# Li-Jinjie/ndp_nmpc_qd

Measured on AMD Instinct MI355X. Metric: NMPC solves/sec (N=20, 1 RTI iter + downwash MLP) at batch, higher is better.
Workload: dtype f64

## Files before the change

### ndp_nmpc_qd_amd/csrc/host.hpp

```cpp
#pragma once
#include <hip/hip_runtime.h>

#include <atomic>
#include <cstdint>
#include <memory>
#include <mutex>
#include <string>
#include <vector>

#include "wave_gfx950.hpp"
#include "cfg_params.hpp"
#include "kern_args.hpp"
#include "rti_table.hpp"
#include "hip_own.hpp"

#define NDP_HIDDEN __attribute__((visibility("hidden")))

using namespace ndp;

struct ndp_handle {
    Stream stream, aux;
    ndp_cfg cfg;
    RtiParams P;
    int lds_per_wave = 0;
    int waves = 4;
    int n_simd = 1024;
    mutable std::atomic<uint64_t> rti_launched{0};
    bool use_queue = false;
    bool queue_auto = false;
    PinnedBuf<unsigned long long> hIpm;
    unsigned long long ipm_seen = 0, steps_seen = 0;
    unsigned queue_launches = 0;
    double *dX = nullptr, *dU = nullptr;
    double *sx0 = nullptr, *sxr = nullptr, *sur = nullptr, *sother = nullptr, *sego = nullptr, *su0 = nullptr;
    float *sf = nullptr;
    int *dStatus = nullptr, *dIters = nullptr;
    const int *lastStatus = nullptr, *lastIters = nullptr;
    double *dRingU = nullptr;
    DevBuf<float> dForce, dFrag;
    DevBuf<double> dKC;
    DevBuf<int> dTables;
    DevBuf<signed char> dAct;
    int sens_level = 0;
    DevBuf<double> dSensU0, dSensU, dSensX;
    DevBuf<double> dPSensXr, dPSensUr, dPSensF;
    DevBuf<double> dVjp;
    DevBuf<int> dVjpSt;
    DevBuf<signed char> dVjpAct;
    DevBuf<double> dClWs;
    DevBuf<int> dFormIndex;
    int form_K = 0, form_edges = 0;
    DevBuf<double> dFormWs;
    DevBuf<float> dFragT, dGwPart;
    DevBuf<float> dFitPart;
    DevBuf<unsigned long long> dTrain;
    DevBuf<double> dThr;
    DevBuf<double> dStamps;
    DevBuf<double> dTraj;
    int traj_seg = 0;
    DevBuf<double> dRingX;
    unsigned long long list_n = 0;
    int segc_par = 0;
    int list_step = 5;
    DevBuf<int> dTickIndex;
    DevBuf<double> dTickThrust;
    bool tick_gate = true;
    const double *tick_remote = nullptr;
    int tick_remote_stride = 6;
    struct TickSlot { bool busy = false, want_u0 = false; } tslot[2];
    DevBuf<double> dRelay;
    DevBuf<double> sThr;
    DevBuf<float> dForceAB[2];
    DevBuf<unsigned long long> dProto;
    Event evFork, evJoin;
    unsigned prefetch_timeout_us = 100000, pf_groups_rti = 1, pf_ntiles = 1;
    DevBuf<unsigned> dQctr;
    DevBuf<int> dQids;
    bool have_mlp = false;
    DevBuf<unsigned char> dIn, dOut;
// ... 185 lines not shown
```

### ndp_nmpc_qd_amd/csrc/kern_args.hpp

```cpp
#pragma once
#include <hip/hip_runtime.h>

#include <stddef.h>

#include <type_traits>

#include "wave_gfx950.hpp"
#include "rti_wave.hpp"

namespace ndp {

struct ThrCfg { double a1, a2, hm, g, R, Q0, Q1, mass; };

struct RingGeom {
    int step, np1;
    __host__ __device__ int ring() const { return step * (np1 - 1) + 1; }
    __host__ __device__ size_t px() const { return (size_t)step * 2 * np1 * 10; }
    __host__ __device__ size_t pu() const { return (size_t)step * 2 * np1 * 4; }
    __host__ __device__ size_t slot(unsigned long long j) const { return (size_t)(j % step) * 2 * np1 + (size_t)((j / step) % np1); }
};

struct RefCfg { int B, N, n_seg; double dt, mass, g, toff; };

struct TickPre {
    RefCfg cf;
    const double *coeff, *tcum, *tseg, *fpt;
    int *seg_hint;
    const double *t;
    double t_all;
    int advance;
    unsigned long long j_new;
    RingGeom rg;
    double *rx, *ru;
    ThrCfg thr;
    double *st;
    const double *vz;
    size_t vz_pitch;
    const double *throttle;
    int est;
    double *pv = nullptr;
    size_t pv_slot = 0;
};

struct BatchPtrs {
    const double *kc;
    const int *tables;
    const double *x0, *xr, *ur;
    const float *f;
    double *X, *U, *u0;
    int *status, *iters;
    double *Xm, *Um;
    double *dbg;
    double *stamps;
    size_t xr_pitch, ur_pitch;
    size_t x0_pitch;
    double *cmd;
    const double *kthr;
    double *thrust_keep;
    double cmd_mass;
    int f_f64;
    signed char *act;
};

struct MlpArgs {
    const float *frag;
    const double *other;
    const double *ego_xy;
    float *force_out;
    double r2;
    int other_stride;
    const int *other_index;
    int other_sys;
    size_t other_pitch;
    size_t ego_pitch;
};

struct QueueArgs {
    unsigned *count;
    int *ids;
    unsigned long long *ipm_total;
};

enum { PF_GROUPS = 8, PF_STRIDE = 512, PF_CUR_M = 0, PF_RTI_C1 = 1 * PF_STRIDE, PF_RTI_C2 = 9 * PF_STRIDE,
       PF_MISSED = 10 * PF_STRIDE, PF_GATE_TIMEOUT = 11 * PF_STRIDE, PF_MLP_DONE = 12 * PF_STRIDE, PF_SLOW = 13 * PF_STRIDE, PF_EPOCH = 14 * PF_STRIDE  };
struct LateArgs {
    unsigned long long *proto;
    const float *F[2];
    unsigned timeout_us;
    unsigned groups_rti, ntiles;
};
__device__ __host__ inline unsigned pf_group_size(unsigned n, unsigned groups, unsigned g) { return n / groups + (g < n % groups ? 1u : 0u); }

enum { SEGC_SLOT = 32, SEGC_PER = 72 };
struct TickArgs {
    const double *coeff, *tcum, *tseg, *fpt;
    const double *segc;
    double *segc_wr;
    int n_seg;
    const double *t;
    double t_all;
    int advance;
    double toff, mass, g;
    unsigned long long j_new;
    size_t new_slot;
    RingGeom rg;
    double *rx, *ru;
    ThrCfg thr;
    double *st;
    const double *vz;
    size_t vz_pitch;
    const double *throttle;
    int est;
};

struct KernArgs {
    RtiParams P;
    BatchPtrs bp;
    int B, lds_per_wave;
    MlpArgs ma;
    QueueArgs qa;
    LateArgs la;
    TickArgs ta;
};
struct SensArgs {
    double *du0 = nullptr, *dU = nullptr, *dX = nullptr;
    int level = 0;
};
// ... 19 lines not shown
```

### ndp_nmpc_qd_amd/csrc/mlp_tile.hpp

```cpp
#pragma once
#include <hip/hip_runtime.h>

#include "mlp_common.hpp"

namespace ndp {

typedef __attribute__((address_space(3))) float *lds_f32;
typedef const __attribute__((address_space(3))) float *lds_cf32;

enum { FR_L1 = 0, FR_B1 = FR_L1 + 12 * 64, FR_B2 = FR_B1 + 128, FR_B3 = FR_B2 + 64, FR_W4 = FR_B3 + 128,
       FR_B4 = FR_W4 + 4 * 128, FR_HF = FR_B4 + 4, FR_REC = 2 * 64 * 8 / 2 ,
       FR_USED = FR_HF + 32 * FR_REC,
       FR_CHUNKS = (FR_USED + 2047) / 2048 * 8, FR_TOTAL = FR_CHUNKS * 256 };
static_assert(FR_HF % 4 == 0 && FR_W4 % 4 == 0, "16-byte alignment of the LDS image");
static_assert(FR_L1 == frag::L1 && FR_B1 == frag::B1 && FR_B2 == frag::B2 && FR_B3 == frag::B3 && FR_W4 == frag::W4 && FR_B4 == frag::B4 &&
              FR_HF == frag::HF && FR_REC == frag::REC && FR_TOTAL == frag::TOTAL, "mlp_common.hpp: frag:: restates this enum for mlp_vjp.hip");


__device__ __forceinline__ void stage_fragments(const float *__restrict__ fr, lds_f32 dst, int tid, int nthreads)
{
    const int wave = __builtin_amdgcn_readfirstlane(tid >> 6), lane = tid & 63, nw = nthreads >> 6;
#pragma unroll
    for (int i = 0; i < FR_CHUNKS; ++i) {
        if (i * nw >= FR_CHUNKS) break;
        const int c = wave + i * nw;
        if ((i + 1) * nw <= FR_CHUNKS || c < FR_CHUNKS)
            __builtin_amdgcn_global_load_lds((const __attribute__((address_space(1))) void *)(fr + c * 256 + lane * 4),
                                             (__attribute__((address_space(3))) void *)(dst + c * 256), 16, 0, 0);
    }
}

__device__ __forceinline__ void load_w(lds_cf32 fr, int rec, int lane, Split2 &w)
{
    const __attribute__((address_space(3))) h16x8 *p = (const __attribute__((address_space(3))) h16x8 *)(fr + FR_HF) + rec * 128 + lane;
    w.hi = p[0]; w.lo = p[64];
}

__device__ __forceinline__ void mlp_tile(lds_cf32 fr, const float zb[3], int lane, float o[3])
{
    typedef float f4_t __attribute__((ext_vector_type(4)));
    const int h = lane >> 5;
    Split2 x1[4][2], x2[2][2];
    f16_t h3[4];
    float bc[16];
#pragma unroll
    for (int ot = 0; ot < 4; ++ot) {
#pragma unroll
        for (int r = 0; r < 16; ++r) bc[r] = fr[FR_B1 + ot * 32 + f0(r) + 4 * h];
        f16_t acc;
#pragma unroll
        for (int r = 0; r < 16; ++r) acc[r] = bc[r];
#pragma unroll
        for (int s = 0; s < 3; ++s)
            acc = __builtin_amdgcn_mfma_f32_32x32x2f32(fr[FR_L1 + (ot * 3 + s) * 64 + lane], zb[s], acc, 0, 0, 0);
#pragma unroll
        for (int r = 0; r < 16; ++r) acc[r] = relu_cap(acc[r]);
        split2(acc, 0, x1[ot][0]);
        split2(acc, 1, x1[ot][1]);
    }
    Split2 wc, wn;
    load_w(fr, 0, lane, wc);
    f16_t acc, accl;
#pragma unroll
    for (int rec = 0; rec < 32; ++rec) {
        const bool l2 = rec < 16;
        const int q = l2 ? rec : rec - 16;
        const int ot = l2 ? q / 8 : q / 4, it = l2 ? (q / 2) % 4 : (q / 2) % 2, s = q % 2;
        const bool first = l2 ? (q % 8 == 0) : (q % 4 == 0), last = l2 ? (q % 8 == 7) : (q % 4 == 3);
        if (rec + 1 < 32) load_w(fr, rec + 1, lane, wn);
        if (first) {
#pragma unroll
            for (int r = 0; r < 16; ++r) {
                acc[r] = fr[(l2 ? FR_B2 : FR_B3) + ot * 32 + f0(r) + 4 * h];
                accl[r] = 0.0f;
            }
        }
#ifdef NDP_DEV_HALF_TILE
        if (!(rec & 1))
#endif
        mm3(wc, l2 ? x1[it][s] : x2[it][s], acc, accl);
        if (last) {
#pragma unroll
            for (int r = 0; r < 16; ++r) {
                const float v = fmaf(accl[r], NDP_LO_INV, acc[r]);
                acc[r] = l2 ? relu_cap(v) : fmaxf(v, 0.0f);
            }
            if (l2) { split2(acc, 0, x2[ot][0]); split2(acc, 1, x2[ot][1]); }
            else h3[ot] = acc;
        }
        wc = wn;
    }
    const __attribute__((address_space(3))) f4_t *w4 = (const __attribute__((address_space(3))) f4_t *)(fr + FR_W4);
    f4_t qc[16], qn[16];
#pragma unroll
    for (int r = 0; r < 16; ++r) qc[r] = w4[f0(r) + 4 * h];
    o[0] = o[1] = o[2] = 0.0f;
#pragma unroll
    for (int it = 0; it < 4; ++it) {
        if (it + 1 < 4) {
#pragma unroll
            for (int r = 0; r < 16; ++r) qn[r] = w4[(it + 1) * 32 + f0(r) + 4 * h];
        }
#pragma unroll
        for (int r = 0; r < 16; ++r) {
#pragma unroll
            for (int c = 0; c < 3; ++c) o[c] = fmaf(qc[r][c], h3[it][r], o[c]);
        }
#pragma unroll
        for (int r = 0; r < 16; ++r) qc[r] = qn[r];
    }
#pragma unroll
    for (int c = 0; c < 3; ++c) o[c] = o[c] + __shfl_xor(o[c], 32, 64) + fr[FR_B4 + c];
}

}
```

### ndp_nmpc_qd_amd/csrc/ndp_hip.hip

```cpp
#include <hip/hip_runtime.h>
#include <hip/hip_ext.h>

#include <sched.h>
#include <stdio.h>

#include <atomic>
#include <chrono>
#include <condition_variable>
#include <cstdlib>
#include <cstring>
#include <memory>
#include <mutex>
#include <new>
#include <string>
#include <thread>
#include <type_traits>
#include <vector>

#include "host.hpp"
#include "cond_qp.hpp"
#include "mlp_tile.hpp"

namespace ndp {

__global__ void queue_reset_kernel(unsigned *count, unsigned long long *ipm_total)
{
    if (threadIdx.x == 0) {
        *ipm_total += *count;
        *count = 0u;
    }
}

}

using namespace ndp;

struct PackJob { unsigned char *dst; const unsigned char *src; size_t len; size_t rows = 0, src_stride = 0; };
enum : size_t { PACK_CHUNK = (size_t)256 << 10 };
struct PackPool {
    std::vector<std::thread> th;
    std::mutex mu;
    std::condition_variable cv;
    std::atomic<const PackJob *> jobs{nullptr};
    std::atomic<int> njobs{0}, next{0}, active{0};
    std::unique_ptr<std::atomic<int>[]> done;
    int done_cap = 0;
    uint64_t gen = 0;
    std::atomic<uint64_t> gen_pub{0};
    bool stop = false;
    static void cpu_relax()
    {
#if !defined(__HIP_DEVICE_COMPILE__) && (defined(__x86_64__) || defined(__i386__))
        __asm__ __volatile__("pause");
#endif
    }

    explicit PackPool(int n)
    {
        for (int i = 0; i < n; ++i) th.emplace_back([this] { work(); });
    }
    ~PackPool()
    {
        { std::lock_guard<std::mutex> lk(mu); stop = true; }
        cv.notify_all();
        for (auto &t : th) t.join();
    }
    bool take_one()
    {
        const int n = njobs.load(std::memory_order_acquire);
        if (n == 0) return false;
        const int i = next.fetch_add(1, std::memory_order_acq_rel);
        if (i >= n) return false;
        const PackJob &j = jobs.load(std::memory_order_relaxed)[i];
        if (j.rows == 0) memcpy(j.dst, j.src, j.len);
// ... 120 lines not shown

int ndp_create(const ndp_cfg *cfg, ndp_handle **out)
{
    if (!cfg || !out) { g_create_err = "ndp_create: null argument"; return -1; }
    *out = nullptr;
    if (cfg->batch < 1 || cfg->N < 2 || slots_for(cfg->N) > 5 || cfg->n_rti < 1 || cfg->qp_precision < 0 || cfg->qp_precision > 6 ||
        cfg->work_queue < 0 || cfg->work_queue > 2 || !(cfg->ts_nmpc > 0.0) || cfg->dt < cfg->ts_nmpc) {
        g_create_err = "ndp_create: need batch >= 1, 2 <= N <= 46, n_rti >= 1, qp_precision in 0..6, work_queue in 0..2, 0 < ts_nmpc <= dt";
        return -2;
    }
    if (cfg->qp_precision >= 5 && (cfg->N % 4 != 0 || cfg->N > 40)) {
        g_create_err = "ndp_create: the condensed study (qp_precision 5 / 6) tiles the 4N x 4N Hessian by 16: N must be a multiple of 4, at most 40";
        return -2;
    }
    if (!as_gamma_holds(*cfg, cfg->Rd)) {
        g_create_err = "ndp_create: as_gamma must be finite and at least 1e8 * max(dt * Rd) when as_iter_max > 0 (a weaker pin does not hold "
                       "its input on the bound)";
        return -2;
    }
    if (cfg->ipm_refine > 0 && (slots_for(cfg->N) > 3 || cfg->qp_precision != 0)) {
        g_create_err = "ndp_create: ipm_refine > 0 is not served for this shape: the refinement path (stiff sweeps + second solves while a STATE bound's "
                       "barrier term exceeds refine_gamma) lives in the three-slot fp64 kernels only (N <= 27, qp_precision 0); the five-slot kernels "
                       "(N >= 28) sit at the register limit without it.  Set ipm_refine = 0: strongly active state bounds at a tight tolerance then "
                       "end in status 4 (never a silent answer)";
        return -2;
    }
    {
        const double ratio = cfg->dt / cfg->ts_nmpc, nearest = (double)(long long)(ratio + 0.5);
        if (ratio - nearest > 1e-9 || nearest - ratio > 1e-9) {
            g_create_err = "ndp_create: dt must be a whole multiple of ts_nmpc (node spacing = every k-th entry of the reference list)";
            return -2;
        }
    }
    int ndev = 0;
    hipError_t e = hipGetDeviceCount(&ndev);
    if (e != hipSuccess || ndev <= cfg->device) {
        g_create_err = std::string("ndp_create: no usable HIP device (") + hipGetErrorString(e) + ")";
        return -3;
    }
    ndp_handle *h = new (std::nothrow) ndp_handle;
    if (!h) return -4;
    h->cfg = *cfg;
    h->P = to_params(*cfg);
    h->list_step = (int)(cfg->dt / cfg->ts_nmpc + 0.5);
    h->lds_per_wave = (lds_doubles(cfg->N) + 1) & ~1;
    if (cfg->qp_precision >= 5) h->lds_per_wave += (cond_extra_doubles(cfg->N) + 1) & ~1;
    const size_t per_wave_bytes = (size_t)h->lds_per_wave * sizeof(double);
    h->waves = 4;
    while (h->waves > 1 && per_wave_bytes * h->waves > 160 * 1024) h->waves >>= 1;
    if (const char *e = getenv("NDP_DEV_WAVES")) {
        const int w = atoi(e);
        if ((w == 1 || w == 2 || w == 4) && w <= h->waves) h->waves = w;
    }
    auto fail = [&](const char *what, hipError_t err) {
        g_create_err = std::string("ndp_create: ") + what + ": " + hipGetErrorString(err);
        ndp_destroy(h);
        return -5;
    };
    if ((e = hipSetDevice(cfg->device)) != hipSuccess) return fail("hipSetDevice", e);
    {
        hipDeviceProp_t prop;
        if ((e = hipGetDeviceProperties(&prop, cfg->device)) != hipSuccess) return fail("hipGetDeviceProperties", e);
        h->n_simd = 4 * prop.multiProcessorCount;
    }
    if (cfg->work_queue == 1 && !(queue_shape(h) && cfg->qp_mode == NDP_QP_AUTO)) {
        g_create_err = "ndp_create: work_queue = 1 needs qp_mode AUTO, qp_precision 0 and (N, n_rti) = (20, 1) or (40, 2)";
        delete h;
        return -2;
    }
    h->queue_auto = cfg->work_queue == 0 && queue_shape(h) && cfg->qp_mode == NDP_QP_AUTO && cfg->N == 20 && cfg->batch >= 2 * h->n_simd;
    h->use_queue = cfg->work_queue == 1 || (cfg->work_queue == 0 && queue_shape(h) && cfg->qp_mode == NDP_QP_AUTO && cfg->N == 40);
    if (h->queue_auto) {
        if ((e = h->hIpm.alloc(64)) != hipSuccess) return fail("hipHostMalloc (work-list counter)", e);
        h->hIpm[0] = h->hIpm[1] = 0;
    }
    if ((e = h->stream.ensure(hipStreamNonBlocking)) != hipSuccess) return fail("hipStreamCreate", e);
    if ((e = h->evLast.ensure(hipEventDisableTiming)) != hipSuccess) return fail("hipEventCreate", e);
    const size_t B = cfg->batch;
    {
        size_t o = 0;
        h->off_x0 = o; o += up256(B * NX * 8);
        h->off_xr = o; o += up256(nxs(h) * 8);
        h->off_ur = o; o += up256(nus(h) * 8);
        h->off_f = o; o += up256(nfs(h) * 8);
        h->off_other = o; o += up256(nxs(h) * 8);
        h->off_ego = o; o += up256(B * 2 * 8);
        h->in_bytes = o;
        o = 0;
        h->off_u0 = o; o += up256(B * NU * 8);
        h->off_st = o; o += up256(B * 4);
        h->off_it = o; o += up256(B * 4);
        h->out_bytes = o;
        h->out_all = h->out_bytes + (nxs(h) + nus(h)) * 8;
    }
    std::string what;
    auto dev = [&](auto &buf, size_t bytes, const char *name) {
        if ((e = buf.alloc(bytes)) != hipSuccess) what = std::string("hipMalloc ") + name;
        return e == hipSuccess;
    };
    if (!dev(h->dForce, nfs(h) * 4, "dForce") || !dev(h->dFrag, FR_TOTAL * 4, "dFrag") || !dev(h->dFragT, FRT_TOTAL * 4, "dFragT") ||
        !dev(h->dGwPart, (size_t)mlp_vjp_groups(h) * NDP_MLP_NPARAM * 4, "dGwPart") || !dev(h->dKC, KC_HOST * 8, "dKC") ||
        !dev(h->dThr, B * 8 * 8, "dThr") || !dev(h->sThr, B * 11 * 8, "sThr") || !dev(h->dRelay, B * 4 * 8, "dRelay") ||
        !dev(h->dQctr, 256, "dQctr") || !dev(h->dQids, B * 4, "dQids") || !dev(h->dAct, act_bytes(h), "dAct") ||
        !dev(h->dTrain, TRAIN_WS_BYTES, "dTrain") ||
        !dev(h->dFitPart, FIT_WS_BYTES, "dFitPart") ||
        !dev(h->dTables, TB_WORDS * 4, "dTables") || !dev(h->dIn, h->in_bytes, "dIn") || !dev(h->dOut, h->out_all, "dOut") ||
// ... 104 lines not shown
    const int N = h->cfg.N, W = h->waves, pr = h->cfg.qp_precision, wi = W == 4 ? 0 : W == 2 ? 1 : 2;
    const bool ref = N == 20 && h->cfg.n_rti == 1;
    if (pr) {
        if (pr >= 3 && N == 40 && h->cfg.n_rti == 2 && W == 2) return pr == 3 ? K40_F32 : K40_BF16;
        return (RtiId)(KPREC1 + pr - 1);
    }
    if (h->sens_level > 0) {
        RtiId id;
        if (phase) id = phase == 2 ? S20_CONS : fused ? S20F_PROD : S20_PROD;
        else if (N == 20 && W == 4) id = fused ? S20F : S20;
        else if (W == 4) id = fused ? SF_4 : S_4;
        else id = fused ? SF_2 : S_2;
        if (!h->dPSensXr) return id;
        switch (id) {
        case S20F_PROD: return P20F_PROD;
        case S20_PROD: return P20_PROD;
        case S20_CONS: return P20_CONS;
        case S20F: return P20F;
        case S20: return P20;
        case SF_4: return PF_4;
        default: return PF_2;
        }
    }
    if (phase == 2) return N == 20 ? K20_CONS : K40_CONS;
    if (phase == 1) {
        if (N != 20) return K40_PROD;
        if (tick) return fused ? K20F_PROD_TICK : K20_PROD_TICK;
        return fused ? K20F_PROD : K20_PROD;
    }
    if (ref && W == 4) {
        if (tick) return fused ? K20F_TICK : K20_TICK;
        return fused ? K20F : prefetched ? K20_LATE : K20;
    }
    if (ref && W == 2) return fused ? K20F_W2 : K20_W2;
    if (N == 40 && h->cfg.n_rti == 2 && W == 2 && !fused) return K40;
    if (fused) return (RtiId)(K3F_4 + wi);
    return (RtiId)((slots_for(N) <= 3 ? K3_4 : K5_4) + wi);
}

int launch_rti(ndp_handle *h, const double *d_x0, const double *d_xr, const double *d_ur, const float *d_f,
               double *d_u0, double *d_dbg, hipStream_t s, const Neigh *nb, const StepOut *so, bool prefetched)
{
    int *d_status = so && so->status ? so->status : h->dStatus, *d_iters = so && so->iters ? so->iters : h->dIters;
    h->lastStatus = d_status; h->lastIters = d_iters;
    BatchPtrs bp{h->dKC, h->dTables, d_x0, d_xr, d_ur, d_f, h->dX, h->dU, d_u0, d_status, d_iters,
                 so ? so->Xm : nullptr, so ? so->Um : nullptr, d_dbg, h->dStamps,
                 so && so->xr_pitch ? so->xr_pitch : (size_t)(h->cfg.N + 1) * NX, so && so->ur_pitch ? so->ur_pitch : (size_t)h->cfg.N * NU, (size_t)NX,
                 so ? so->cmd : nullptr, so ? so->kthr : nullptr, so ? so->thrust_keep : nullptr, h->cfg.mass, so && so->f_f64 ? 1 : 0,
                 h->dAct};
    const bool fused = nb && nb->other;
    MlpArgs ma{fused ? h->dFrag : nullptr, fused ? nb->other : nullptr, fused ? nb->ego_xy : nullptr, h->dForce,
               h->cfg.r_horiz * h->cfg.r_horiz, fused ? nb->stride : NX, fused ? nb->index : nullptr, fused ? peer_mapped(nb->other) : 0,
               fused && nb->pitch ? nb->pitch : (size_t)(h->cfg.N + 1) * (fused ? nb->stride : NX), fused && nb->ego_pitch ? nb->ego_pitch : (size_t)2};
    QueueArgs qa{h->dQctr, h->dQids, reinterpret_cast<unsigned long long *>(h->dQctr + 16)};
    LateArgs la{prefetched ? h->dProto : nullptr, {h->dForceAB[0], h->dForceAB[1]}, h->prefetch_timeout_us,
                h->pf_groups_rti, h->pf_ntiles};
    KernArgs ka{h->P, bp, h->cfg.batch, h->lds_per_wave, ma, qa, la, so && so->tick ? *so->tick : TickArgs{}};
    SensArgs sa{h->dSensU0, h->sens_level >= 2 ? h->dSensU : nullptr, h->sens_level >= 2 ? h->dSensX : nullptr, h->sens_level};
    const bool tick1 = so && so->tick;
    const int pr = h->cfg.qp_precision;
    const bool q = h->use_queue && !d_dbg && !prefetched;
    h->last_step_tracked = false;
    if (h->track_steps) {
        hipStreamCaptureStatus cs = hipStreamCaptureStatusNone;
        if (hipStreamIsCapturing(s, &cs) != hipSuccess) { (void)hipGetLastError(); cs = hipStreamCaptureStatusNone; }
        if (cs != hipStreamCaptureStatusNone) {
            h->err = "tracked control steps (ndp_track_steps) cannot be launched on a stream that is being captured: switch tracking off "
                     "and order the exchange through the stream (ndp_xchg_begin's after_stream)";
            return -15;
        }
    }
    int rc = begin_timing(h, s, 0, true);
    if (rc) return rc;
    const bool ext_timing = h->timing_open && !q && !pr && !(so && so->done) && !h->track_steps;
    if (h->timing_open && !ext_timing) NDP_HIP(h, hipEventRecord(h->events.back().a, s));
    if (pr && fused) { h->err = "qp_precision != 0 supports f / no disturbance only (run ndp_downwash first)"; return -12; }
    hipEvent_t stop = nullptr;
    if (so && so->done) stop = so->done;
    else if (h->track_steps) { stop = h->stepDone[++h->step_seq & 3]; h->last_step_tracked = true; }
    if (h->sens_level > 0 && (prefetched || tick1)) { h->err = "launch_rti: the late-force and tick forms have no sensitivity kernel"; return -2; }
    launch_kern(h, rti_pick(h, fused, tick1, prefetched, q ? 1 : 0), s, ka, sa, ext_timing ? h->events.back().a : nullptr,
                ext_timing ? h->events.back().b : q || pr ? nullptr : stop);
    if (ext_timing) h->timing_open = false;
    NDP_HIP(h, hipGetLastError());
    if (q) {
        KernArgs kc = ka;
        kc.bp.f = fused ? h->dForce : d_f;
        kc.ma.frag = nullptr; kc.ma.other = nullptr;
        if (h->cfg.n_rti == 1 && h->cfg.as_iter_max <= 0) kc.P.qp_mode = QP_IPM_ALWAYS;
        launch_kern(h, rti_pick(h, fused, tick1, prefetched, 2), s, kc, sa);
        NDP_HIP(h, hipGetLastError());
        if (stop) hipExtLaunchKernelGGL(queue_reset_kernel, dim3(1), dim3(64), 0, s, nullptr, stop, 0, h->dQctr.get(), qa.ipm_total);
        else hipLaunchKernelGGL(queue_reset_kernel, dim3(1), dim3(64), 0, s, h->dQctr, qa.ipm_total);
        NDP_HIP(h, hipGetLastError());
    } else if (pr && stop) NDP_HIP(h, hipEventRecord(stop, s));
    const int rce = end_timing(h, s);
    queue_policy(h, s);
    return rce;
}

bool can_fuse(const ndp_handle *h)
{
    return h->cfg.qp_precision == 0 && h->cfg.N + 1 <= 32 && slots_for(h->cfg.N) <= 3 &&
           (size_t)h->lds_per_wave * sizeof(double) * h->waves >= FR_TOTAL * sizeof(float);
}

// ... 669 lines not shown
```

### ndp_nmpc_qd_amd/csrc/rti_kernel_body.inc

```
    static_assert(!(FUSED && QMODE == 2), "the consumer reads the force the producer left in global memory");
    static_assert(!TICK || (QMODE <= 1 && NC > 0 && PREC == 0), "the one-launch tick exists for the compile-time horizon's in-place and producer forms");
#ifndef NDP_NO_KERNARG_WARM
    {
        typedef const __attribute__((address_space(4))) unsigned *kptr;
        kptr kp = (kptr)__builtin_amdgcn_kernarg_segment_ptr();
        unsigned acc = 0;
#pragma unroll
        for (unsigned o = 0; o < (unsigned)sizeof(KernArgs); o += 64) acc |= kp[o / 4];
        asm volatile("" : : "s"(acc));
    }
#endif
    const RtiParams &P = ka.P;
    const BatchPtrs &bp = ka.bp;
    const MlpArgs &ma = ka.ma;
    const QueueArgs &qa = ka.qa;
    const int B = ka.B;
    const int wave = (int)(threadIdx.x >> 6);
    if (!FUSED && (QMODE == 0 || QMODE == 3) && ka.la.proto) {
        if (threadIdx.x == 0) wg_done = 0;
        __syncthreads();
    }
    int inst_raw = __builtin_amdgcn_readfirstlane((int)blockIdx.x * WAVES + wave);
    if (QMODE == 2) {
        const int n = (int)*qa.count;
        if (inst_raw >= n) return;
        inst_raw = __builtin_amdgcn_readfirstlane(qa.ids[inst_raw]);
    }
    const bool active = inst_raw < B;
    if (!FUSED && !active) return;
    const int inst = active ? inst_raw : B - 1;
    const int N = NC ? NC : P.N;
    const size_t nf = (size_t)(N + 1) * 3;
    RtiIo io;
    bind_instance(io, bp, inst, N);
    if (NSLOT <= 3 && (QMODE == 0 || QMODE == 3)) io.ipm_ctr = qa.ipm_total;
    if (NSLOT <= 3 && QMODE != 2 && blockIdx.x == 0 && threadIdx.x == 0 && qa.ipm_total)
        __hip_atomic_fetch_add(qa.ipm_total + 1, 1ull, __ATOMIC_RELAXED, __HIP_MEMORY_SCOPE_AGENT);
    if (!FUSED && (QMODE == 0 || QMODE == 3) && ka.la.proto) {
        const LateArgs &la = ka.la;
        const unsigned long long t = la.proto[PF_RTI_C2] / la.groups_rti + 1;
        const unsigned g = blockIdx.x % la.groups_rti;
        const unsigned np1 = (unsigned)N + 1, row0 = (unsigned)inst * np1;
        io.f_late = la.F[t & 1] + (size_t)inst * nf;
        io.late_flag = la.proto + PF_EPOCH + (t & 1) * la.ntiles + row0 / 32;
        io.late_flag2 = la.proto + PF_EPOCH + (t & 1) * la.ntiles + (row0 + np1 - 1) / 32;
        io.late_want = t;
        io.late_ready = la.proto[PF_MLP_DONE] >= t ? 1 : 0;
        io.late_timeout_us = la.timeout_us;
        io.late_missed = reinterpret_cast<int *>(la.proto + PF_MISSED);
        io.late_slow = reinterpret_cast<int *>(la.proto + PF_SLOW);
        io.late_cnt = reinterpret_cast<unsigned *>(la.proto + PF_RTI_C1 + PF_STRIDE * g);
        io.late_done_word = la.proto + PF_RTI_C2;
        io.late_gsize = pf_group_size(gridDim.x, la.groups_rti, g);
        io.late_group = (void *)((size_t)(unsigned)(size_t)(__attribute__((address_space(3))) unsigned *)&wg_done + 1);
        const int left = B - (int)blockIdx.x * WAVES;
        io.late_group_size = (unsigned)(left < WAVES ? left : WAVES);
    }
    const int lpw = NC ? ((lds_doubles(NC) + 1) & ~1) : ka.lds_per_wave;
    WaveGfx950::lds_ptr lds = (WaveGfx950::lds_ptr)(smem + (size_t)wave * lpw);
    using WB = std::conditional_t<PREC == 3, WaveGfx950F32, std::conditional_t<PREC == 4, WaveGfx950BF16, WaveGfx950>>;
    using Prog = RtiWave<WB, NSLOT, NC, true, NRC, (PREC >= 3 ? 0 : PREC), QMODE == 3, (PREC == 5 ? 1 : (PREC == 6 ? 2 : 0))>;
    if (NDP_RARELY(io.stamps && (threadIdx.x & 63u) == 0)) {
        io.stamps[12] = (double)__builtin_amdgcn_s_memrealtime();
        io.stamps[14] = (double)__builtin_amdgcn_s_memtime();
    }
    int orow = inst;
    bool wg_nb = true;
    if (FUSED && ma.other_index) {
        int any = 0;
#pragma unroll
        for (int w = 0; w < WAVES; ++w) {
            const int iw = (int)blockIdx.x * WAVES + w;
            any |= (ma.other_index[iw < B ? iw : B - 1] >= 0) ? 1 : 0;
        }
        orow = __builtin_amdgcn_readfirstlane(ma.other_index[inst]);
        asm volatile("" : : "s"(orow));
        wg_nb = __builtin_amdgcn_readfirstlane(any) != 0;
    }
    const bool advance = TICK && ka.ta.advance != 0;
    TickEarly te;
    if (TICK && NDP_RARELY(io.stamps && (threadIdx.x & 63u) == 0)) io.stamps[16] = (double)__builtin_amdgcn_s_memtime();
    if (TICK && advance) {
        te = tick_early(ka.ta, inst, FUSED && wg_nb ? orow : -1, (int)(threadIdx.x & 63u));
        __builtin_amdgcn_sched_barrier(0);
    }
    if (TICK && NDP_RARELY(io.stamps && (threadIdx.x & 63u) == 0)) io.stamps[22] = (double)__builtin_amdgcn_s_memtime();
    typename Prog::InBuf inb;
    double x0v;
    Prog::issue_first(P, io, inb, x0v);
    __builtin_amdgcn_sched_barrier(0);
    if (TICK && NDP_RARELY(io.stamps && (threadIdx.x & 63u) == 0)) io.stamps[23] = (double)__builtin_amdgcn_s_memtime();
    double x_new[10], u_new[4], nb_new[6], seg_fill = 0.0, seg_cfill = 0.0;
    int seg_refill = 0;
    if (TICK && !(FUSED && wg_nb) && advance) {
        tick_arrived(te);
        seg_fill = tick_new_point(ka.ta, te, inst, (int)(threadIdx.x & 63u), active, x_new, u_new, nb_new, seg_refill, seg_cfill, io.stamps);
#pragma unroll
        for (int i = 0; i < 10; ++i) io.xrN[i] = x_new[i];
        io.have_xrN = 1;
    }
    if (FUSED && !wg_nb) {
        if (!active) return;
        const int lane = (int)(threadIdx.x & 63u);
        const LdsMap m = make_map(N);
        if (lane < 3 * (N + 1)) {
            lds[m.TF + lane] = 0.0;
            ma.force_out[inst * nf + lane] = 0.0f;
        }
        if (3 * (N + 1) > 64 && lane + 64 < 3 * (N + 1)) {
            lds[m.TF + lane + 64] = 0.0;
            ma.force_out[inst * nf + lane + 64] = 0.0f;
        }
        WaveGfx950::sync();
        io.f = nullptr;
        io.f_in_lds = 1;
    } else if (FUSED) {
        const int lane = (int)(threadIdx.x & 63u), j = lane & 31, h = lane >> 5;
        const int np1 = N + 1;
        const int st = ma.other_stride;
        const double *oth = ma.other + (size_t)(orow < 0 ? 0 : orow) * ma.other_pitch;
        const double *exy = ma.ego_xy ? ma.ego_xy + (size_t)inst * ma.ego_pitch : oth;
        const int osys = ma.other_sys;
        const double g_ox = ld_other(oth, osys), g_oy = ld_other(oth + 1, osys), g_ex = exy[0], g_ey = exy[1];
        const int jr = j < np1 ? j : np1 - 1;
        float zb[3], o[3];
        typedef double d2_t __attribute__((ext_vector_type(2)));
        constexpr int ZR = NC ? (3 * (NC + 1) + 63) / 64 : 2;
        d2_t dv[ZR], ev[ZR];
#pragma unroll
        for (int t = 0; t < ZR; ++t) {
            const int l3 = lane + 64 * t, r3 = l3 / 3, c3 = l3 - 3 * r3, rc = r3 < np1 ? r3 : np1 - 1;
            dv[t] = ld_other2(oth + (size_t)rc * st + 2 * c3, osys);
            ev[t] = *(const d2_t *)(io.xr + (size_t)rc * NX + 2 * c3);
        }
        const LdsMap m = make_map(N);
        if (NDP_RARELY(io.dbg && lane == 0)) io.dbg[m.total + 9] = (double)__builtin_amdgcn_s_memtime();
        if (NDP_RARELY(io.stamps && lane == 0)) io.stamps[9] = (double)__builtin_amdgcn_s_memtime();
        lds_f32 wl = (lds_f32)smem;
        if (TICK) tick_arrived(te);
        stage_fragments(ma.frag, wl, (int)threadIdx.x, 64 * WAVES);
        if (TICK && advance) {
            seg_fill = tick_new_point(ka.ta, te, inst, lane, active, x_new, u_new, nb_new, seg_refill, seg_cfill, io.stamps);
#pragma unroll
            for (int i = 0; i < 10; ++i) io.xrN[i] = x_new[i];
            io.have_xrN = 1;
#pragma unroll
            for (int t = 0; t < ZR; ++t) {
                const int l3 = lane + 64 * t, r3 = l3 / 3, c3 = l3 - 3 * r3;
                if (r3 == N) {
                    dv[t][0] = c3 == 0 ? nb_new[0] : (c3 == 1 ? nb_new[2] : nb_new[4]);
                    dv[t][1] = c3 == 0 ? nb_new[1] : (c3 == 1 ? nb_new[3] : nb_new[5]);
                    ev[t][0] = c3 == 0 ? x_new[0] : (c3 == 1 ? x_new[2] : x_new[4]);
                    ev[t][1] = c3 == 0 ? x_new[1] : (c3 == 1 ? x_new[3] : x_new[5]);
                }
            }
        }
        __syncthreads();
        const double g_o[2] = {g_ox, g_oy}, g_e[2] = {g_ex, g_ey};
        const bool open = orow >= 0 && (ma.ego_xy ? gate_open(g_o, g_e, ma.r2) : true);
        {
            float fx[ZR], fy[ZR];
#pragma unroll
            for (int t = 0; t < ZR; ++t) { fx[t] = (float)(dv[t][0] - ev[t][0]); fy[t] = (float)(dv[t][1] - ev[t][1]); }
#pragma unroll
            for (int s = 0; s < 3; ++s) {
                const int src = 3 * jr + s, sl = (src & 63) << 2;
                float vx = __int_as_float(__builtin_amdgcn_ds_bpermute(sl, __float_as_int(fx[0])));
                float vy = __int_as_float(__builtin_amdgcn_ds_bpermute(sl, __float_as_int(fy[0])));
                if (ZR > 1) {
                    const float wx = __int_as_float(__builtin_amdgcn_ds_bpermute(sl, __float_as_int(fx[ZR - 1])));
                    const float wy = __int_as_float(__builtin_amdgcn_ds_bpermute(sl, __float_as_int(fy[ZR - 1])));
                    if (src >= 64) { vx = wx; vy = wy; }
                }
                zb[s] = h ? vy : vx;
            }
        }
        if (NDP_RARELY(io.stamps && lane == 0)) io.stamps[11] = (double)__builtin_amdgcn_s_memtime();
        o[0] = o[1] = o[2] = 0.0f;
        if (__builtin_amdgcn_readfirstlane((int)open)) mlp_tile(wl, zb, lane, o);
        __syncthreads();
        if (!active) return;
        if (NDP_RARELY(io.dbg && lane == 0)) io.dbg[m.total + 10] = (double)__builtin_amdgcn_s_memtime();
        if (NDP_RARELY(io.stamps && lane == 0)) io.stamps[10] = (double)__builtin_amdgcn_s_memtime();
        if (j < np1 && h == 0) {
#pragma unroll
            for (int c = 0; c < 3; ++c) {
                const float v = open ? o[c] : 0.0f;
                lds[m.TF + j * 3 + c] = (double)v;
                ma.force_out[inst * nf + j * 3 + c] = v;
            }
        }
        WaveGfx950::sync();
        io.f = nullptr;
        io.f_in_lds = 1;
    }
    if (TICK && advance && active) tick_cache_store(ka.ta, te, inst, (int)(threadIdx.x & 63u), seg_refill, seg_fill, seg_cfill);
    if (TICK && ka.ta.est && active) io.kthr = tick_estimator(ka.ta, inst, B, (int)(threadIdx.x & 63u));
    bool deferred;
    if constexpr (SENS) {
        const SensIo so{sa.du0 + (size_t)inst * sens_u0_pitch(), sa.dU ? sa.dU + (size_t)inst * sens_u_pitch(N) : nullptr,
                        sa.dX ? sa.dX + (size_t)inst * sens_x_pitch(N) : nullptr, sa.level};
        if constexpr (PSENS) {
            const PSensIo po{pa.dxr + (size_t)inst * psens_xr_pitch(N), pa.dur + (size_t)inst * psens_ur_pitch(N), pa.df + (size_t)inst * psens_f_pitch(N)};
            deferred = Prog::template run<QMODE == 1, QMODE == 0 || QMODE == 3, true, true>(P, io, lds, inb, x0v, &so, &po);
        } else {
            deferred = Prog::template run<QMODE == 1, QMODE == 0 || QMODE == 3, true>(P, io, lds, inb, x0v, &so);
        }
    } else {
        deferred = Prog::template run<QMODE == 1, QMODE == 0 || QMODE == 3>(P, io, lds, inb, x0v);
    }
    if (NDP_RARELY(io.stamps && (threadIdx.x & 63u) == 0)) {
        io.stamps[13] = (double)__builtin_amdgcn_s_memrealtime();
        io.stamps[15] = (double)__builtin_amdgcn_s_memtime();
    }
    if (QMODE == 1 && deferred && (threadIdx.x & 63u) == 0) {
        const unsigned s = __hip_atomic_fetch_add(qa.count, 1u, __ATOMIC_RELAXED, __HIP_MEMORY_SCOPE_AGENT);
        qa.ids[s] = inst;
    }
```

### ndp_nmpc_qd_amd/csrc/rti_kernels.hip

```cpp
#include <hip/hip_runtime.h>
#include <hip/hip_ext.h>

#include <type_traits>

#include "wave_gfx950.hpp"
#include "cfg_params.hpp"
#include "cond_qp.hpp"
#include "host.hpp"
#include "mlp_common.hpp"
#include "mlp_tile.hpp"
#include "ref_point.hpp"
#include "tick_wave.hpp"

namespace ndp {

__device__ __forceinline__ void bind_instance(RtiIo &io, const BatchPtrs &bp, int inst, int N)
{
    const size_t nx = (size_t)(N + 1) * NX, nu = (size_t)N * NU, nf = (size_t)(N + 1) * 3;
    io.x0 = bp.x0 + (size_t)inst * bp.x0_pitch;
    io.xr = bp.xr + inst * bp.xr_pitch;
    io.ur = bp.ur + inst * bp.ur_pitch;
    io.f = bp.f ? bp.f + inst * nf * (bp.f_f64 ? 2 : 1) : nullptr;
    io.f_is_f64 = bp.f_f64;
    io.X = bp.X + inst * nx;
    io.U = bp.U + inst * nu;
    io.Xm = bp.Xm ? bp.Xm + inst * nx : nullptr;
    io.Um = bp.Xm ? bp.Um + inst * nu : nullptr;
    io.u0 = bp.u0 + (size_t)inst * NU;
    io.status = bp.status + inst;
    io.iters = bp.iters + inst;
    io.dbg = bp.dbg;
    io.f_in_lds = 0;
    io.kc = bp.kc;
    io.tables = bp.tables;
    io.stamps = bp.stamps ? bp.stamps + (size_t)inst * NDP_NSTAMP : nullptr;
    io.act = bp.act ? bp.act + (size_t)inst * act_pitch(N) : nullptr;
    if (NDP_RARELY(bp.cmd != nullptr)) {
        io.cmd = bp.cmd + (size_t)inst * NU;
        io.thrust_keep = bp.thrust_keep + inst;
        io.kthr = bp.kthr[inst];
        io.cmd_mass = bp.cmd_mass;
    }
}

#ifndef NDP_RTI_ATTR
#define NDP_RTI_ATTR
#endif
template <int NSLOT, int WAVES, bool FUSED, int NC = 0, int PREC = 0, int NRC = (NC ? 1 : 0), int QMODE = 0, bool TICK = false>
__global__ __launch_bounds__(64 * WAVES) NDP_RTI_ATTR void rti_kernel(KernArgs ka)
{
    constexpr bool SENS = false, PSENS = false;
    const SensArgs sa{};
    const PSensArgs pa{};
    extern __shared__ __attribute__((aligned(16))) double smem[];
    __shared__ unsigned wg_done;
#include "rti_kernel_body.inc"
}

template <int WAVES, bool FUSED, int NC, int QMODE>
__global__ __launch_bounds__(64 * WAVES) void rti_sens_kernel(KernArgs ka, SensArgs sa)
{
    constexpr int NSLOT = 3, PREC = 0, NRC = NC ? 1 : 0;
    constexpr bool TICK = false, SENS = true, PSENS = false;
// ... 352 lines not shown
```

Baseline: 46.11 million.

## Add gate-aware instance placement with paired-wave MLP tile split

Adds an opt-in placement mode (NDP_DEV_PLACE=1) where each workgroup first evaluates the downwash gate for all instances, ballots the open ones, and remaps instances so open-gate MLP work is spread evenly across workgroups. When a group has few open instances, an idle wave pairs with an open one and the MLP tile is split in halves across the two waves, exchanging intermediate activations through LDS with barriers. This targets load imbalance where some waves run the MLP while others idle, at the cost of extra global loads, ballot/scan work, and more LDS and barriers in the fused path. Default is off, but the PAIR template path also changes the default kernel (mlp_tile_w<true>, late params).

```diff
diff --git a/ndp_nmpc_qd_amd/csrc/host.hpp b/ndp_nmpc_qd_amd/csrc/host.hpp
--- a/ndp_nmpc_qd_amd/csrc/host.hpp
+++ b/ndp_nmpc_qd_amd/csrc/host.hpp
@@ -25,6 +25,7 @@
     int lds_per_wave = 0;
     int waves = 4;
     int n_simd = 1024;
+    bool place = false;
     mutable std::atomic<uint64_t> rti_launched{0};
     bool use_queue = false;
     bool queue_auto = false;
diff --git a/ndp_nmpc_qd_amd/csrc/kern_args.hpp b/ndp_nmpc_qd_amd/csrc/kern_args.hpp
--- a/ndp_nmpc_qd_amd/csrc/kern_args.hpp
+++ b/ndp_nmpc_qd_amd/csrc/kern_args.hpp
@@ -73,6 +73,7 @@
     int other_sys;
     size_t other_pitch;
     size_t ego_pitch;
+    int place = 0;
 };
 
 struct QueueArgs {
diff --git a/ndp_nmpc_qd_amd/csrc/mlp_tile.hpp b/ndp_nmpc_qd_amd/csrc/mlp_tile.hpp
--- a/ndp_nmpc_qd_amd/csrc/mlp_tile.hpp
+++ b/ndp_nmpc_qd_amd/csrc/mlp_tile.hpp
@@ -36,68 +36,116 @@
     w.hi = p[0]; w.lo = p[64];
 }
 
-__device__ __forceinline__ void mlp_tile(lds_cf32 fr, const float zb[3], int lane, float o[3])
+enum { TILE_NONE = 0, TILE_WHOLE = 1, TILE_FIRST = 2, TILE_SECOND = 3 };
+enum { TW_L1 = 1, TW_G0 = 1 << 1, TW_IT0 = 1 << 7, TW_FIRST = 1 << 11, TW_SECOND = 1 << 12, TW_END = 1 << 13,
+       TW_WHOLE = TW_L1 | 63 * TW_G0 | 15 * TW_IT0 | TW_END,
+       TW_OF_FIRST = TW_L1 | (1 | 4 | 8) * TW_G0 | 3 * TW_IT0 | TW_FIRST,
+       TW_OF_SECOND = TW_L1 | (2 | 16 | 32) * TW_G0 | 12 * TW_IT0 | TW_SECOND | TW_END };
+enum { XCH_X2 = 2 * 2 * 64 * 4 , XCH_O = 2 * XCH_X2, XCH_TOTAL = XCH_O + 3 * 64 + 64 };
+static_assert(XCH_TOTAL % 4 == 0, "16-byte alignment of the second pair's exchange area");
+
+__device__ __forceinline__ void xch_put(lds_f32 x, int lane, const Split2 v[2])
+{
+    __attribute__((address_space(3))) h16x8 *p = (__attribute__((address_space(3))) h16x8 *)x + lane;
+    p[0] = v[0].hi; p[64] = v[0].lo; p[128] = v[1].hi; p[192] = v[1].lo;
+}
+__device__ __forceinline__ void xch_get(lds_f32 x, int lane, Split2 v[2])
+{
+    const __attribute__((address_space(3))) h16x8 *p = (const __attribute__((address_space(3))) h16x8 *)x + lane;
+    v[0].hi = p[0]; v[0].lo = p[64]; v[1].hi = p[128]; v[1].lo = p[192];
+}
+
+template <bool PAIR>
+__device__ __forceinline__ void mlp_tile_w(lds_cf32 fr, const float zb[3], int lane, float o[3], int role = TILE_WHOLE, lds_f32 xch = nullptr)
 {
     typedef float f4_t __attribute__((ext_vector_type(4)));
     const int h = lane >> 5;
+    const unsigned work = !PAIR || role == TILE_WHOLE ? TW_WHOLE : role == TILE_FIRST ? TW_OF_FIRST : role == TILE_SECOND ? TW_OF_SECOND : 0u;
     Split2 x1[4][2], x2[2][2];
     f16_t h3[4];
     float bc[16];
+    if (!PAIR || (work & TW_L1)) {
 #pragma unroll
-    for (int ot = 0; ot < 4; ++ot) {
+        for (int ot = 0; ot < 4; ++ot) {
 #pragma unroll
-        for (int r = 0; r < 16; ++r) bc[r] = fr[FR_B1 + ot * 32 + f0(r) + 4 * h];
-        f16_t acc;
+            for (int r = 0; r < 16; ++r) bc[r] = fr[FR_B1 + ot * 32 + f0(r) + 4 * h];
+            f16_t acc;
 #pragma unroll
-        for (int r = 0; r < 16; ++r) acc[r] = bc[r];
+            for (int r = 0; r < 16; ++r) acc[r] = bc[r];
 #pragma unroll
-        for (int s = 0; s < 3; ++s)
-            acc = __builtin_amdgcn_mfma_f32_32x32x2f32(fr[FR_L1 + (ot * 3 + s) * 64 + lane], zb[s], acc, 0, 0, 0);
+            for (int s = 0; s < 3; ++s)
+                acc = __builtin_amdgcn_mfma_f32_32x32x2f32(fr[FR_L1 + (ot * 3 + s) * 64 + lane], zb[s], acc, 0, 0, 0);
 #pragma unroll
-        for (int r = 0; r < 16; ++r) acc[r] = relu_cap(acc[r]);
-        split2(acc, 0, x1[ot][0]);
-        split2(acc, 1, x1[ot][1]);
+            for (int r = 0; r < 16; ++r) acc[r] = relu_cap(acc[r]);
+            split2(acc, 0, x1[ot][0]);
+            split2(acc, 1, x1[ot][1]);
+        }
     }
     Split2 wc, wn;
-    load_w(fr, 0, lane, wc);
+    if (!PAIR) load_w(fr, 0, lane, wc);
     f16_t acc, accl;
 #pragma unroll
-    for (int rec = 0; rec < 32; ++rec) {
-        const bool l2 = rec < 16;
-        const int q = l2 ? rec : rec - 16;
-        const int ot = l2 ? q / 8 : q / 4, it = l2 ? (q / 2) % 4 : (q / 2) % 2, s = q % 2;
-        const bool first = l2 ? (q % 8 == 0) : (q % 4 == 0), last = l2 ? (q % 8 == 7) : (q % 4 == 3);
-        if (rec + 1 < 32) load_w(fr, rec + 1, lane, wn);
-        if (first) {
+    for (int g = 0; g < 6; ++g) {
+        const bool l2 = g < 2;
+        const int ot = l2 ? g : g - 2, n = l2 ? 8 : 4, rec0 = l2 ? 8 * ot : 16 + 4 * ot;
+        if (PAIR && g == 2) {
+            if (work & TW_FIRST) xch_put(xch, lane, x2[0]);
+            if (work & TW_SECOND) xch_put(xch + XCH_X2, lane, x2[1]);
+            __syncthreads();
+            if (work & TW_FIRST) xch_get(xch + XCH_X2, lane, x2[1]);
+            if (work & TW_SECOND) xch_get(xch, lane, x2[0]);
+        }
+        if (PAIR && !(work & (TW_G0 << g))) continue;
+        if (PAIR) load_w(fr, rec0, lane, wc);
 #pragma unroll
-            for (int r = 0; r < 16; ++r) {
-                acc[r] = fr[(l2 ? FR_B2 : FR_B3) + ot * 32 + f0(r) + 4 * h];
-                accl[r] = 0.0f;
+        for (int q = 0; q < n; ++q) {
+            const int rec = rec0 + q, it = q / 2, s = q % 2;
+            if (PAIR ? q + 1 < n : rec + 1 < 32) load_w(fr, rec + 1, lane, wn);
+            if (q == 0) {
+#pragma unroll
+                for (int r = 0; r < 16; ++r) {
+                    acc[r] = fr[(l2 ? FR_B2 : FR_B3) + ot * 32 + f0(r) + 4 * h];
+                    accl[r] = 0.0f;
+                }
             }
+            mm3(wc, l2 ? x1[it][s] : x2[it][s], acc, accl);
+            if (q == n - 1) {
+#pragma unroll
+                for (int r = 0; r < 16; ++r) {
+                    const float v = fmaf(accl[r], NDP_LO_INV, acc[r]);
+                    acc[r] = l2 ? relu_cap(v) : fmaxf(v, 0.0f);
+                }
+                if (l2) { split2(acc, 0, x2[ot][0]); split2(acc, 1, x2[ot][1]); }
+                else h3[ot] = acc;
+            }
+            wc = wn;
         }
-#ifdef NDP_DEV_HALF_TILE
-        if (!(rec & 1))
-#endif
-        mm3(wc, l2 ? x1[it][s] : x2[it][s], acc, accl);
-        if (last) {
-#pragma unroll
-            for (int r = 0; r < 16; ++r) {
-                const float v = fmaf(accl[r], NDP_LO_INV, acc[r]);
-                acc[r] = l2 ? relu_cap(v) : fmaxf(v, 0.0f);
-            }
-            if (l2) { split2(acc, 0, x2[ot][0]); split2(acc, 1, x2[ot][1]); }
-            else h3[ot] = acc;
-        }
-        wc = wn;
     }
     const __attribute__((address_space(3))) f4_t *w4 = (const __attribute__((address_space(3))) f4_t *)(fr + FR_W4);
     f4_t qc[16], qn[16];
+    if (!PAIR) {
 #pragma unroll
-    for (int r = 0; r < 16; ++r) qc[r] = w4[f0(r) + 4 * h];
+        for (int r = 0; r < 16; ++r) qc[r] = w4[f0(r) + 4 * h];
+    }
     o[0] = o[1] = o[2] = 0.0f;
 #pragma unroll
     for (int it = 0; it < 4; ++it) {
-        if (it + 1 < 4) {
+        if (PAIR && it == 2) {
+            if (work & TW_FIRST) {
+#pragma unroll
+                for (int c = 0; c < 3; ++c) xch[XCH_O + c * 64 + lane] = o[c];
+            }
+            __syncthreads();
+            if (work & TW_SECOND) {
+#pragma unroll
+                for (int c = 0; c < 3; ++c) o[c] = xch[XCH_O + c * 64 + lane];
+            }
+        }
+        if (PAIR && !(work & (TW_IT0 << it))) continue;
+        if (PAIR) {
+#pragma unroll
+            for (int r = 0; r < 16; ++r) qc[r] = w4[it * 32 + f0(r) + 4 * h];
+        } else if (it + 1 < 4) {
 #pragma unroll
             for (int r = 0; r < 16; ++r) qn[r] = w4[(it + 1) * 32 + f0(r) + 4 * h];
         }
@@ -106,11 +154,17 @@
 #pragma unroll
             for (int c = 0; c < 3; ++c) o[c] = fmaf(qc[r][c], h3[it][r], o[c]);
         }
+        if (!PAIR) {
 #pragma unroll
-        for (int r = 0; r < 16; ++r) qc[r] = qn[r];
+            for (int r = 0; r < 16; ++r) qc[r] = qn[r];
+        }
     }
+    if (!PAIR || (work & TW_END)) {
 #pragma unroll
-    for (int c = 0; c < 3; ++c) o[c] = o[c] + __shfl_xor(o[c], 32, 64) + fr[FR_B4 + c];
+        for (int c = 0; c < 3; ++c) o[c] = o[c] + __shfl_xor(o[c], 32, 64) + fr[FR_B4 + c];
+    }
 }
 
+__device__ __forceinline__ void mlp_tile(lds_cf32 fr, const float zb[3], int lane, float o[3]) { mlp_tile_w<false>(fr, zb, lane, o); }
+
 }
diff --git a/ndp_nmpc_qd_amd/csrc/ndp_hip.hip b/ndp_nmpc_qd_amd/csrc/ndp_hip.hip
--- a/ndp_nmpc_qd_amd/csrc/ndp_hip.hip
+++ b/ndp_nmpc_qd_amd/csrc/ndp_hip.hip
@@ -20,6 +20,7 @@
 #include "host.hpp"
 #include "cond_qp.hpp"
 #include "mlp_tile.hpp"
+#include "place_select.hpp"
 
 namespace ndp {
 
@@ -246,6 +247,7 @@
         const int w = atoi(e);
         if ((w == 1 || w == 2 || w == 4) && w <= h->waves) h->waves = w;
     }
+    if (const char *e = getenv("NDP_DEV_PLACE")) h->place = atoi(e) == 1;
     auto fail = [&](const char *what, hipError_t err) {
         g_create_err = std::string("ndp_create: ") + what + ": " + hipGetErrorString(err);
         ndp_destroy(h);
@@ -456,6 +458,8 @@
     MlpArgs ma{fused ? h->dFrag : nullptr, fused ? nb->other : nullptr, fused ? nb->ego_xy : nullptr, h->dForce,
                h->cfg.r_horiz * h->cfg.r_horiz, fused ? nb->stride : NX, fused ? nb->index : nullptr, fused ? peer_mapped(nb->other) : 0,
                fused && nb->pitch ? nb->pitch : (size_t)(h->cfg.N + 1) * (fused ? nb->stride : NX), fused && nb->ego_pitch ? nb->ego_pitch : (size_t)2};
+    ma.place = h->place && fused && h->waves == 4 && h->cfg.batch <= h->n_simd && h->cfg.batch <= PLACE_MAX_B &&
+               (size_t)h->lds_per_wave * sizeof(double) * h->waves >= (FR_TOTAL + 2 * XCH_TOTAL) * sizeof(float) + PLACE_LDS_BYTES;
     QueueArgs qa{h->dQctr, h->dQids, reinterpret_cast<unsigned long long *>(h->dQctr + 16)};
     LateArgs la{prefetched ? h->dProto : nullptr, {h->dForceAB[0], h->dForceAB[1]}, h->prefetch_timeout_us,
                 h->pf_groups_rti, h->pf_ntiles};
diff --git a/ndp_nmpc_qd_amd/csrc/place_select.hpp b/ndp_nmpc_qd_amd/csrc/place_select.hpp
--- /dev/null
+++ b/ndp_nmpc_qd_amd/csrc/place_select.hpp
@@ -0,0 +1,48 @@
+#pragma once
+
+#if defined(__HIPCC__) || defined(__CUDACC__)
+#define NDP_PLACE_HD __host__ __device__
+#else
+#define NDP_PLACE_HD
+#endif
+
+namespace ndp {
+
+enum { PLACE_WORDS = 16, PLACE_MAX_B = 64 * PLACE_WORDS,
+       PLACE_LDS_BYTES = PLACE_WORDS * 8 + 4 * 4 * 4 };
+
+NDP_PLACE_HD inline int place_kth_set(unsigned long long w, int k)
+{
+    unsigned v = (unsigned)w;
+    int pos = 0;
+    const int c32 = __builtin_popcount(v);
+    if (k >= c32) { k -= c32; v = (unsigned)(w >> 32); pos = 32; }
+    for (int sh = 16; sh; sh >>= 1) {
+        const int c = __builtin_popcount(v & ((1u << sh) - 1u));
+        if (k >= c) { k -= c; v >>= sh; pos += sh; }
+    }
+    return pos;
+}
+
+NDP_PLACE_HD inline int place_lane(unsigned long long w, int incl, int j, int p, int n_open, int B)
+{
+    if (p >= B) return -1;
+    const bool want_open = p < n_open;
+    const int k = want_open ? p : p - n_open;
+    const int left = B - 64 * j, vc = left < 0 ? 0 : (left > 64 ? 64 : left);
+    const int c = __builtin_popcountll(w);
+    const int cls_incl = want_open ? incl : 64 * j + vc - incl, cls_c = want_open ? c : vc - c;
+    const int k_in = k - (cls_incl - cls_c);
+    if (k_in < 0 || k_in >= cls_c) return -1;
+    const unsigned long long valid = vc >= 64 ? ~0ull : (1ull << vc) - 1ull;
+    return 64 * j + place_kth_set(want_open ? w : ~w & valid, k_in);
+}
+
+NDP_PLACE_HD inline int place_open_in_group(int n_open, int G, int g, int waves)
+{
+    int k = 0;
+    for (int w = 0; w < waves; ++w) k += (w * G + g < n_open) ? 1 : 0;
+    return k;
+}
+
+}
diff --git a/ndp_nmpc_qd_amd/csrc/rti_kernel_body.inc b/ndp_nmpc_qd_amd/csrc/rti_kernel_body.inc
--- a/ndp_nmpc_qd_amd/csrc/rti_kernel_body.inc
+++ b/ndp_nmpc_qd_amd/csrc/rti_kernel_body.inc
@@ -26,6 +26,75 @@
         if (inst_raw >= n) return;
         inst_raw = __builtin_amdgcn_readfirstlane(qa.ids[inst_raw]);
     }
+    constexpr bool PAIR = FUSED && !TICK && !SENS && WAVES == 4 && QMODE <= 1;
+    int tile_how = -1, tile_inst = inst_raw;
+    if constexpr (PAIR) if (__builtin_amdgcn_readfirstlane(ma.place) != 0) {
+        typedef const __attribute__((address_space(4))) KernArgs *kargs_ptr;
+        kargs_ptr kargs = (kargs_ptr)__builtin_amdgcn_kernarg_segment_ptr();
+        asm volatile("" : "+s"(kargs));
+        const __attribute__((address_space(4))) MlpArgs &mp = kargs->ma;
+        int tile_role = TILE_NONE, pair = 0;
+        const int lane = (int)(threadIdx.x & 63u), wv = __builtin_amdgcn_readfirstlane(wave);
+        lds_f32 wl = (lds_f32)smem;
+        constexpr int GR = PLACE_MAX_B / (64 * WAVES);
+        int gi[GR], grow[GR];
+        double gox[GR], goy[GR], gex[GR], gey[GR];
+#pragma unroll
+        for (int t = 0; t < GR; ++t) {
+            const int i = (int)threadIdx.x + 64 * WAVES * t;
+            gi[t] = i < B ? i : B - 1;
+            grow[t] = mp.other_index ? mp.other_index[gi[t]] : gi[t];
+        }
+#pragma unroll
+        for (int t = 0; t < GR; ++t) {
+            gox[t] = goy[t] = gex[t] = gey[t] = 0.0;
+            if (mp.ego_xy) {
+                const double *go = mp.other + (size_t)(grow[t] < 0 ? 0 : grow[t]) * mp.other_pitch, *ge = mp.ego_xy + (size_t)gi[t] * mp.ego_pitch;
+                gox[t] = ld_other(go, mp.other_sys); goy[t] = ld_other(go + 1, mp.other_sys);
+                gex[t] = ge[0]; gey[t] = ge[1];
+            }
+        }
+        stage_fragments(mp.frag, wl, (int)threadIdx.x, 64 * WAVES);
+        __attribute__((address_space(3))) unsigned long long *gw = (__attribute__((address_space(3))) unsigned long long *)(wl + FR_TOTAL + 2 * XCH_TOTAL);
+#pragma unroll
+        for (int t = 0; t < GR; ++t) {
+            const double g_o[2] = {gox[t], goy[t]}, g_e[2] = {gex[t], gey[t]};
+            const bool op = (int)threadIdx.x + 64 * WAVES * t < B && grow[t] >= 0 && (mp.ego_xy ? gate_open(g_o, g_e, mp.r2) : true);
+            const unsigned long long word = __ballot(op);
+            if (lane == 0) gw[WAVES * t + wv] = word;
+        }
+        __syncthreads();
+        static_assert(WAVES * PLACE_WORDS == 64, "one row of 16 lanes per slot of the workgroup");
+        const int jw = lane & 15, q = lane >> 4, G = (int)gridDim.x, g = (int)blockIdx.x;
+        const unsigned long long word = gw[jw];
+        int incl = __builtin_popcountll(word);
+        incl += __builtin_amdgcn_update_dpp(0, incl, 0x111, 0xF, 0xF, true);
+        incl += __builtin_amdgcn_update_dpp(0, incl, 0x112, 0xF, 0xF, true);
+        incl += __builtin_amdgcn_update_dpp(0, incl, 0x114, 0xF, 0xF, true);
+        incl += __builtin_amdgcn_update_dpp(0, incl, 0x118, 0xF, 0xF, true);
+        const int n_open = __builtin_amdgcn_readfirstlane(__builtin_amdgcn_update_dpp(0, incl, 0x150 + 15, 0xF, 0xF, true));
+        const int found = place_lane(word, incl, jw, q * G + g, n_open, B);
+        __attribute__((address_space(3))) int *res = (__attribute__((address_space(3))) int *)(gw + PLACE_WORDS) + WAVES * wv;
+        if (jw == 0) res[q] = B;
+        if (found >= 0) res[q] = found;
+        int slot[WAVES];
+#pragma unroll
+        for (int w = 0; w < WAVES; ++w) slot[w] = __builtin_amdgcn_readfirstlane(res[w]);
+        const int k = place_open_in_group(n_open, G, g, WAVES);
+        int mate = wv;
+        if (2 * k <= WAVES) {
+            if (wv < k) { tile_role = TILE_SECOND; pair = wv; }
+            else if (wv < 2 * k) { tile_role = TILE_FIRST; pair = wv - k; mate = wv - k; }
+        } else if (wv < k) tile_role = TILE_WHOLE;
+        inst_raw = tile_inst = slot[0];
+#pragma unroll
+        for (int w = 1; w < WAVES; ++w) {
+            if (wv == w) inst_raw = slot[w];
+            if (mate == w) tile_inst = slot[w];
+        }
+        tile_how = tile_role + 4 * pair;
+    }
+    const bool placed = PAIR && tile_how >= 0;
     const bool active = inst_raw < B;
     if (!FUSED && !active) return;
     const int inst = active ? inst_raw : B - 1;
@@ -64,18 +133,21 @@
         io.stamps[12] = (double)__builtin_amdgcn_s_memrealtime();
         io.stamps[14] = (double)__builtin_amdgcn_s_memtime();
     }
-    int orow = inst;
+    const int tin = PAIR && (tile_how & 3) == TILE_FIRST && placed ? tile_inst : inst;
+    int orow = tin;
     bool wg_nb = true;
     if (FUSED && ma.other_index) {
         int any = 0;
-#pragma unroll
-        for (int w = 0; w < WAVES; ++w) {
-            const int iw = (int)blockIdx.x * WAVES + w;
-            any |= (ma.other_index[iw < B ? iw : B - 1] >= 0) ? 1 : 0;
-        }
-        orow = __builtin_amdgcn_readfirstlane(ma.other_index[inst]);
+        if (!placed) {
+#pragma unroll
+            for (int w = 0; w < WAVES; ++w) {
+                const int iw = (int)blockIdx.x * WAVES + w;
+                any |= (ma.other_index[iw < B ? iw : B - 1] >= 0) ? 1 : 0;
+            }
+        }
+        orow = __builtin_amdgcn_readfirstlane(ma.other_index[tin]);
         asm volatile("" : : "s"(orow));
-        wg_nb = __builtin_amdgcn_readfirstlane(any) != 0;
+        wg_nb = placed || __builtin_amdgcn_readfirstlane(any) != 0;
     }
     const bool advance = TICK && ka.ta.advance != 0;
     TickEarly te;
@@ -127,18 +199,19 @@
         typedef double d2_t __attribute__((ext_vector_type(2)));
         constexpr int ZR = NC ? (3 * (NC + 1) + 63) / 64 : 2;
         d2_t dv[ZR], ev[ZR];
+        const double *txr = PAIR ? bp.xr + tin * bp.xr_pitch : io.xr;
 #pragma unroll
         for (int t = 0; t < ZR; ++t) {
             const int l3 = lane + 64 * t, r3 = l3 / 3, c3 = l3 - 3 * r3, rc = r3 < np1 ? r3 : np1 - 1;
             dv[t] = ld_other2(oth + (size_t)rc * st + 2 * c3, osys);
-            ev[t] = *(const d2_t *)(io.xr + (size_t)rc * NX + 2 * c3);
+            ev[t] = *(const d2_t *)(txr + (size_t)rc * NX + 2 * c3);
         }
         const LdsMap m = make_map(N);
         if (NDP_RARELY(io.dbg && lane == 0)) io.dbg[m.total + 9] = (double)__builtin_amdgcn_s_memtime();
         if (NDP_RARELY(io.stamps && lane == 0)) io.stamps[9] = (double)__builtin_amdgcn_s_memtime();
         lds_f32 wl = (lds_f32)smem;
         if (TICK) tick_arrived(te);
-        stage_fragments(ma.frag, wl, (int)threadIdx.x, 64 * WAVES);
+        if (!placed) stage_fragments(ma.frag, wl, (int)threadIdx.x, 64 * WAVES);
         if (TICK && advance) {
             seg_fill = tick_new_point(ka.ta, te, inst, lane, active, x_new, u_new, nb_new, seg_refill, seg_cfill, io.stamps);
 #pragma unroll
@@ -155,9 +228,10 @@
                 }
             }
         }
-        __syncthreads();
+        if (!placed) __syncthreads();
         const double g_o[2] = {g_ox, g_oy}, g_e[2] = {g_ex, g_ey};
-        const bool open = orow >= 0 && (ma.ego_xy ? gate_open(g_o, g_e, ma.r2) : true);
+        const bool open = placed ? (tile_how & 3) == TILE_SECOND || (tile_how & 3) == TILE_WHOLE
+                                 : orow >= 0 && (ma.ego_xy ? gate_open(g_o, g_e, ma.r2) : true);
         {
             float fx[ZR], fy[ZR];
 #pragma unroll
@@ -177,7 +251,10 @@
         }
         if (NDP_RARELY(io.stamps && lane == 0)) io.stamps[11] = (double)__builtin_amdgcn_s_memtime();
         o[0] = o[1] = o[2] = 0.0f;
-        if (__builtin_amdgcn_readfirstlane((int)open)) mlp_tile(wl, zb, lane, o);
+        if constexpr (PAIR) {
+            const int role = placed ? tile_how & 3 : (__builtin_amdgcn_readfirstlane((int)open) ? TILE_WHOLE : TILE_NONE);
+            mlp_tile_w<true>(wl, zb, lane, o, __builtin_amdgcn_readfirstlane(role), wl + FR_TOTAL + (placed ? tile_how >> 2 : 0) * XCH_TOTAL);
+        } else if (__builtin_amdgcn_readfirstlane((int)open)) mlp_tile(wl, zb, lane, o);
         __syncthreads();
         if (!active) return;
         if (NDP_RARELY(io.dbg && lane == 0)) io.dbg[m.total + 10] = (double)__builtin_amdgcn_s_memtime();
@@ -207,7 +284,9 @@
             deferred = Prog::template run<QMODE == 1, QMODE == 0 || QMODE == 3, true>(P, io, lds, inb, x0v, &so);
         }
     } else {
-        deferred = Prog::template run<QMODE == 1, QMODE == 0 || QMODE == 3>(P, io, lds, inb, x0v);
+        const RtiParams *Pr = &P;
+        if constexpr (PAIR) Pr = (const RtiParams *)WaveGfx950::late_params(P);
+        deferred = Prog::template run<QMODE == 1, QMODE == 0 || QMODE == 3>(*Pr, io, lds, inb, x0v);
     }
     if (NDP_RARELY(io.stamps && (threadIdx.x & 63u) == 0)) {
         io.stamps[13] = (double)__builtin_amdgcn_s_memrealtime();
diff --git a/ndp_nmpc_qd_amd/csrc/rti_kernels.hip b/ndp_nmpc_qd_amd/csrc/rti_kernels.hip
--- a/ndp_nmpc_qd_amd/csrc/rti_kernels.hip
+++ b/ndp_nmpc_qd_amd/csrc/rti_kernels.hip
@@ -9,6 +9,7 @@
 #include "host.hpp"
 #include "mlp_common.hpp"
 #include "mlp_tile.hpp"
+#include "place_select.hpp"
 #include "ref_point.hpp"
 #include "tick_wave.hpp"
 
```

Measured after the change: 43.14 million. -6.4%, worse.
